# boyuanf/tensorflow_train_distributed

Hardware: AMD Instinct MI355X
Metric: images/sec (whole node) ResNet-50 bf16 MirroredStrategy at 1/2/4/8 MI355X (higher is better)
Workload: dtype bf16; 1 GPU; model=ResNet-50 v1.5, global_batch=1024, per_gpu_batch=1024, image_size=224, parallelism=dp1, optimizer=momentum-SGD 0.9, wd 5e-5, fp32 master, precision=bf16, hipgraph=True

## Files before the change

tensorflow_train_distributed_amd/csrc/kernels/conv3_halo.hip:

```cpp
#include "stream_epi.h"

namespace ttdk {
namespace {
namespace c3 {

constexpr int THR = 512;
constexpr int NW = THR / 64;

struct Pro {
  const bf16_t* x;
  const bf16_t* x2;
  const uint8_t* mask;
  const float* s;
  const float* b;
  bf16_t* side;
  uint8_t* side_mask;
};

__device__ __forceinline__ void load8f(const float* p, float (&d)[8]) {
  const f32x4_t a = *reinterpret_cast<const f32x4_t*>(p), c = *reinterpret_cast<const f32x4_t*>(p + 4);
#pragma unroll
  for (int j = 0; j < 4; ++j) {
    d[j] = a[j];
    d[4 + j] = c[j];
  }
}

template <int CP>
__device__ __forceinline__ int slot_chunk(int q) { return (q >> 3) % CP; }
template <int CP>
__device__ __forceinline__ int slot_pix(int q) { return (q & 7) + 8 * (q / (8 * CP)); }

template <int SCHED>
__device__ __forceinline__ int fresh(int tid) {
  if constexpr (SCHED != 0) {
    asm volatile("" : "+v"(tid));
    __builtin_assume(tid >= 0 && tid < THR);
  }
  return tid;
}

template <int SCHED>
__device__ __forceinline__ void frag_fence() {
  if constexpr (SCHED != 0) __builtin_amdgcn_sched_barrier(0);
}

template <int C, int BN, int TH, int W, int PRO, bool FLIP, int WM, int SCHED>
__global__ __launch_bounds__(THR, 1) void conv3_kernel(Pro pa, const bf16_t* __restrict__ w, EpiParams E, int H,
                                                      int N, int tiles, int nslices) {
  constexpr int BM = TH * W;
  constexpr int HR = TH + 2, HC = W + 2;
  constexpr int CP = C / 8;
  constexpr int KT = 9 * C;
  constexpr int WN = NW / WM;
  constexpr int WR = BM / WM, WC = BN / WN;
  constexpr int TM = WR / 16, TN = WC / 16;
  constexpr int NPIX = HR * HC;
  constexpr int NCH = ((NPIX + 7) / 8) * 8 * CP;
  constexpr int NA = (NCH + THR - 1) / THR;
  constexpr int SB = BN * KT * 2;
  constexpr int REG = ((NPIX * 16 + 255) / 256) * 256;
  constexpr int SH = CP * REG;
  constexpr int PITCH = BN * 2 + 16;
  constexpr int SE = BM * PITCH + NW * 3 * BN * 4;
  constexpr int SAE = SH > SE ? SH : SE;
  static_assert(C % 64 == 0 && BN % 32 == 0 && WR % 16 == 0 && WC % 16 == 0, "tile shape");
  static_assert(THR % (8 * CP) == 0, "fixed channel chunk per thread");
  static_assert(SB + SAE <= 160 * 1024, "LDS budget");
  __shared__ __attribute__((aligned(16))) char smem[SB + SAE];
  char* const sB = smem;
  char* const sA = smem + SB;

  const int b = blockIdx.x;
  const int G = gridDim.x / nslices;
  const int xcd = b & 7, rq = b >> 3;
  const int slice = rq % nslices;
  const int per_xcd = G / 8;
  const int g = xcd * per_xcd + rq / nslices;
  const int n0 = slice * BN;
  const int tid = threadIdx.x, lane = tid & 63, wave = tid >> 6;
  const int wm = wave / WN, wn = wave % WN;
  const int tiles_per_img = H / TH;

  for (int q = tid; q < BN * (KT / 8); q += THR) {
    const int row = q / (KT / 8), kk = q % (KT / 8);
    const int tap = kk / CP, cc = kk % CP;
    const int n = n0 + row;
    const int src_tap = FLIP ? 8 - tap : tap;
    const uint4 v = n < N ? ldg16(w + (static_cast<long long>(n) * 9 + src_tap) * C + cc * 8) : make_uint4(0, 0, 0, 0);
    *reinterpret_cast<uint4*>(sB + (kk >> 3) * (BN * 128) + kmaj_off(row, kk & 7)) = v;
  }

  const int ac = slot_chunk<CP>(tid);
  const bool write_side = slice == 0 && pa.side != nullptr;

  const char* abase[TM];
#pragma unroll
  for (int a = 0; a < TM; ++a) {
    const int i = wm * WR + a * 16 + (lane & 15);
    abase[a] = sA + (lane >> 4) * REG + ((i / W) * HC + (i % W)) * 16;
  }

  uint4 ra[NA], rx[PRO == 2 ? NA : 1];
  uint32_t rm[(NA + 3) / 4];
  auto load_tile = [&](int t) {
    const int img = t / tiles_per_img, h0 = (t % tiles_per_img) * TH;
    const int ft = fresh<SCHED>(tid);
#pragma unroll
    for (int i = 0; i < (NA + 3) / 4; ++i) rm[i] = 0;
#pragma unroll
    for (int i = 0; i < NA; ++i) {
      const int pix = slot_pix<CP>(ft + THR * i);
      const int hr = pix / HC, hc = pix % HC;
      const int h = h0 - 1 + hr, x = hc - 1;
      const bool ok = pix < NPIX && h >= 0 && h < H && x >= 0 && x < W;
      const long long off = ((static_cast<long long>(img) * H + h) * W + x) * C + ac * 8;
      ra[i] = ok ? ldg16(pa.x + off) : make_uint4(0, 0, 0, 0);
      if constexpr (PRO == 2) {
        rx[i] = ok ? ldg16(pa.x2 + off) : make_uint4(0, 0, 0, 0);
        rm[i >> 2] |= static_cast<uint32_t>((ok && pa.mask) ? pa.mask[off >> 3] : 0xffu) << (8 * (i & 3));
      }
    }
  };
  auto stage_tile = [&](int t) {
    const int img = t / tiles_per_img, h0 = (t % tiles_per_img) * TH;
    float k0[8], k1[8], k2[8];
    if constexpr (PRO == 1) {
      load8f(pa.s + ac * 8, k0);
      load8f(pa.b + ac * 8, k1);
    } else if constexpr (PRO == 2) {
      load8f(pa.s + ac * 8, k0);
      load8f(pa.s + C + ac * 8, k1);
      load8f(pa.s + 2 * C + ac * 8, k2);
    }
    const int ft = fresh<SCHED>(tid);
#pragma unroll
    for (int i = 0; i < NA; ++i) {
      const int pix = slot_pix<CP>(ft + THR * i);
      if (ft + THR * i >= NCH) break;
      const int hr = pix / HC, hc = pix % HC;
      const int h = h0 - 1 + hr, x = hc - 1;
      const bool ok = h >= 0 && h < H && x >= 0 && x < W;
      const bool interior = ok && hr >= 1 && hr <= TH;
      const long long off = ((static_cast<long long>(img) * H + h) * W + x) * C + ac * 8;
      uint4 v = ra[i];
      if constexpr (PRO == 1) {
        float f[8];
        unpack8(ra[i], f);
#pragma unroll
        for (int j = 0; j < 8; ++j) f[j] = relu(f[j] * k0[j] + k1[j]);
        v = ok ? pack8(f) : make_uint4(0, 0, 0, 0);
        if (write_side && interior) {
          *reinterpret_cast<uint4*>(pa.side + off) = v;
          if (pa.side_mask) {
            const uint32_t wv[4] = {v.x, v.y, v.z, v.w};
            uint32_t mb = 0;
#pragma unroll
            for (int j = 0; j < 8; ++j) {
              const uint32_t hb = (wv[j >> 1] >> (16 * (j & 1))) & 0xffffu;
              mb |= ((hb & 0x7fffu) != 0 && !(hb & 0x8000u) ? 1u : 0u) << j;
            }
            pa.side_mask[off >> 3] = static_cast<uint8_t>(mb);
          }
        }
      } else if constexpr (PRO == 2) {
        float gq[8], yf[8];
        unpack8(ra[i], gq);
        const uint32_t mb = rm[i >> 2] >> (8 * (i & 3));
#pragma unroll
        for (int j = 0; j < 8; ++j) gq[j] = (mb >> j) & 1u ? gq[j] : 0.f;
        unpack8(rx[i], yf);
#pragma unroll
        for (int j = 0; j < 8; ++j) gq[j] = k0[j] * gq[j] + k1[j] * yf[j] + k2[j];
        v = ok ? pack8(gq) : make_uint4(0, 0, 0, 0);
        if (write_side && interior) *reinterpret_cast<uint4*>(pa.side + off) = v;
      }
      *reinterpret_cast<uint4*>(sA + ac * REG + pix * 16) = v;
    }
  };

  int t = g;
  if (t < tiles) load_tile(t);
  for (; t < tiles; t += G) {
    stage_tile(t);
    __syncthreads();
    if (t + G < tiles) load_tile(t + G);
    f32x4_t acc[TM][TN];
#pragma unroll
    for (int a = 0; a < TM; ++a)
#pragma unroll
      for (int c = 0; c < TN; ++c) acc[a][c] = f32x4_t{0.f, 0.f, 0.f, 0.f};
#pragma unroll
    for (int tap = 0; tap < 9; ++tap) {
      const int tq = (tap / 3) * HC + (tap % 3);
#pragma unroll
      for (int kc = 0; kc < C / 32; ++kc) {
        const int kglob = tap * C + kc * 32;
        const char* pB = sB + (kglob >> 6) * (BN * 128);
        const int kchunk = ((kglob & 63) >> 3) + (lane >> 4);
        bf16x8_t af[TM], bfr[TN];
#pragma unroll
        for (int c = 0; c < TN; ++c) {
          bfr[c] = lds_read_b128(pB + kmaj_off(wn * WC + c * 16 + (lane & 15), kchunk));
          frag_fence<SCHED>();
        }
#pragma unroll
        for (int a = 0; a < TM; ++a) {
          af[a] = lds_read_b128(abase[a] + kc * 4 * REG + tq * 16);
          frag_fence<SCHED>();
        }
#pragma unroll
        for (int a = 0; a < TM; ++a)
#pragma unroll
          for (int c = 0; c < TN; ++c) acc[a][c] = __builtin_amdgcn_mfma_f32_16x16x32_bf16(bfr[c], af[a], acc[a][c], 0, 0, 0);
        frag_fence<SCHED>();
      }
    }
    __syncthreads();
    sepi::stage_acc<TM, TN, WR, WC, PITCH>(sA, acc, wm, wn, lane, epi_alpha(E));
    __syncthreads();
    constexpr int ECPR = BN / 8;
    constexpr int RPP = THR / ECPR;
    const int m0 = t * BM;
    const int c = tid % ECPR, r0 = tid / ECPR;
    const int n = n0 + c * 8;
    const bool nfull = n + 8 <= N;
    const bool vst = nfull && (E.ldo & 7) == 0;
    float bias8[8], s8[8], q8[8], r8[8];
#pragma unroll
    for (int j = 0; j < 8; ++j) {
      bias8[j] = (E.bias && n + j < N) ? E.bias[n + j] : 0.f;
      s8[j] = q8[j] = r8[j] = 0.f;
    }
    const int M = tiles * BM;
    if (E.beta || E.residual || E.by)
      epi_rows<BM, RPP, PITCH, true, 2>(E, sA, c, r0, n, m0, M, N, vst, vst, bias8, s8, q8, r8);
    else
      epi_rows<BM, RPP, PITCH, false>(E, sA, c, r0, n, m0, M, N, vst, vst, bias8, s8, q8, r8);
    if (E.stat)
      sepi::tile_stats<BN, NW, THR, ECPR>(E, reinterpret_cast<float*>(sA + BM * PITCH), s8, q8, r8, c, lane, wave, tid,
                                          n0, N, t);
    else
      __syncthreads();
  }
}

template <int C, int BN, int TH, int W, int PRO, bool FLIP, int WM, int SCHED>
hipError_t launch(const Pro& pa, const bf16_t* w, const EpiParams& E, int Nimg, int H, int N, hipStream_t st) {
  const int nsl = N / BN;
  const int tiles = Nimg * (H / TH);
  int per_xcd = big::device_cus() / (8 * nsl);
  if (per_xcd < 1) per_xcd = 1;
  const int need = ceil_div(tiles, 8);
  if (per_xcd > need) per_xcd = need;
  hipLaunchKernelGGL((conv3_kernel<C, BN, TH, W, PRO, FLIP, WM, SCHED>), dim3(8 * nsl * per_xcd), dim3(THR), 0, st, pa, w,
                     E, H, N, tiles, nsl);
  return hipGetLastError();
}

inline int pick_th(int C, int N, int W, int pro) {
  if (C == 64 && N == 64 && W == 56) return pro == 2 ? 4 : 8;
  return 0;
}

template <int PRO, bool FLIP, int SCHED>
hipError_t dispatch(const Pro& pa, const bf16_t* w, const EpiParams& E, int Nimg, int H, int W, int C, int N,
                    hipStream_t st) {
  if (C == 64 && N == 64 && W == 56) {
    if constexpr (PRO == 2) return launch<64, 64, 4, 56, PRO, FLIP, 2, SCHED>(pa, w, E, Nimg, H, N, st);
    else return launch<64, 64, 8, 56, PRO, FLIP, 4, SCHED>(pa, w, E, Nimg, H, N, st);
  }
  return hipErrorInvalidValue;
}

}

namespace c3s {

constexpr int THR = 512;
constexpr int NW = THR / 64;

__device__ __forceinline__ void dma16(const void* src, uint32_t lds_) {
  const uint32_t lds = __builtin_amdgcn_readfirstlane(lds_);
  unsigned keep;
  asm volatile("s_mov_b32 %0, m0\n\ts_mov_b32 m0, %2\n\ts_nop 0\n\tglobal_load_lds_dwordx4 %1, off\n\ts_mov_b32 m0, %0"
               : "=&s"(keep) : "v"(src), "s"(lds) : "memory");
}
__device__ __forceinline__ uint32_t lds_addr(const char* p) {
  typedef __attribute__((address_space(3))) const char lds_char_t;
  return (uint32_t)(size_t)(lds_char_t*)(p);
}

template <int N>
__device__ __forceinline__ void wait_vm() {
  asm volatile("s_waitcnt vmcnt(%0)" ::"n"(N) : "memory");
}
__device__ __forceinline__ void wait_vm_upto(int n) {
  switch (n) {
    case 1: wait_vm<1>(); break;
    case 2: wait_vm<2>(); break;
    case 3: wait_vm<3>(); break;
    default: wait_vm<0>(); break;
  }
}

template <int C, int BN, int TR, int H, int W, int PRO, bool FLIP, int SCHED>
__global__ __launch_bounds__(THR, 1) void conv3s_kernel(c3::Pro pa, const bf16_t* __restrict__ w, EpiParams E,
                                                       int rows_total, int N, int tiles) {
  constexpr int WM = 2, WN = NW / WM;
  constexpr int BM = TR * W;
  constexpr int WR = BM / WM, WC = BN / WN;
  constexpr int TM = WR / 16, TN = WC / 16;
  constexpr int HS = TR + 4;
  constexpr int HC = W + 2;
  constexpr int NPIX = HS * HC;
  constexpr int CP = C / 8;
  constexpr int NCH = ((NPIX + 7) / 8) * 8 * CP;
  constexpr int NA = (NCH + THR - 1) / THR;
  constexpr int REG = ((NPIX * 16 + 255) / 256) * 256;
  constexpr int SH = CP * REG;
  constexpr int SBT = BN * C * 2;
  constexpr int PITCH = BN * 2 + 16;
  constexpr int SE = BM * PITCH + NW * 3 * BN * 4;
  constexpr int SAE = SH > SE ? SH : SE;
  constexpr int NDMA = SBT / 16 / THR;
  static_assert(PRO != 2 && C % 64 == 0 && BN % (16 * WN) == 0 && WR % 16 == 0 && TR <= H, "tile shape");
  static_assert(THR % (8 * CP) == 0 && SBT % (16 * THR) == 0, "staging / DMA mapping");
  static_assert(SAE + 2 * SBT <= 160 * 1024, "LDS budget");
  __shared__ __attribute__((aligned(16))) char smem[SAE + 2 * SBT];
  char* const sA = smem;
  char* const sBb = smem + SAE;

  const int b = blockIdx.x;
  const int G = gridDim.x;
  const int g = (b & 7) * (G / 8) + (b >> 3);
  const int tid = threadIdx.x, lane = tid & 63, wave = tid >> 6;
  const int wm = wave / WN, wn = wave % WN;
  const int ac = c3::slot_chunk<CP>(tid);
  const bool write_side = pa.side != nullptr;
  const int nimg = rows_total / H;

  const bf16_t* wsrc[NDMA];
#pragma unroll
  for (int i = 0; i < NDMA; ++i) {
    const int L = (i * NW + wave) * 64 + lane;
    const int sub = L / (BN * 8), p = L % (BN * 8), row = p >> 3, j = p & 7;
    const int sc = j ^ ((row >> 1) & 7);
    wsrc[i] = w + static_cast<long long>(row) * 9 * C + (sub * 8 + sc) * 8;
  }
  auto dma_tap = [&](int tap, int buf) {
    const int stap = FLIP ? 8 - tap : tap;
    char* dst = sBb + buf * SBT;
#pragma unroll
    for (int i = 0; i < NDMA; ++i) {
      if constexpr (SCHED != 0) {
        int off = stap * C;
        asm volatile("" : "+s"(off));
        dma16(wsrc[i] + off, lds_addr(dst + (i * NW + wave) * 1024));
      } else {
        const int L = (i * NW + wave) * 64 + lane;
        const int sub = L / (BN * 8), p = L % (BN * 8), row = p >> 3, j = p & 7;
        const int sc = j ^ ((row >> 1) & 7);
        dma16(w + (static_cast<long long>(row) * 9 + stap) * C + (sub * 8 + sc) * 8,
              lds_addr(dst + (i * NW + wave) * 1024));
      }
    }
  };
  struct Geo {
    int i0, h0, n0, n1;
  };
  auto geo = [&](int t) {
    Geo q;
    const int R0 = t * TR, R1 = min(R0 + TR, rows_total);
    q.i0 = R0 / H;
    q.h0 = R0 - q.i0 * H;
    q.n0 = min(R1, (q.i0 + 1) * H) - R0;
    q.n1 = R1 - R0 - q.n0;
    return q;
  };
  auto slot_src = [&](const Geo& q, int s, int& img, int& h, bool& interior) {
    if (s < q.n0 + 2) {
      img = q.i0;
      h = q.h0 - 1 + s;
      interior = s >= 1 && s <= q.n0;
      return true;
    }
    const int u = s - (q.n0 + 2);
    img = q.i0 + 1;
    h = u - 1;
    interior = u >= 1 && u <= q.n1;
    return q.n1 > 0 && u < q.n1 + 2;
  };

  uint4 ra[NA];
  auto load_slot = [&](const Geo& q, int ft, int i) {
    const int qq = ft + THR * i;
    const int pix = c3::slot_pix<CP>(qq);
    const int s = pix / HC, x = pix % HC - 1;
    int img, h;
    bool interior;
    const bool ok = qq < NCH && slot_src(q, s, img, h, interior) && h >= 0 && h < H && x >= 0 && x < W;
    const long long off = ((static_cast<long long>(img) * H + h) * W + x) * C + ac * 8;
    ra[i] = ldg16(ok ? pa.x + off : reinterpret_cast<const bf16_t*>(big::g_zero));
  };
  auto load_tile = [&](int t) {
    const Geo q = geo(t);
    const int ft = c3::fresh<SCHED>(tid);
#pragma unroll
    for (int i = 0; i < NA; ++i) load_slot(q, ft, i);
  };
  auto stage_tile = [&](int t) {
    const Geo q = geo(t);
    float k0[8], k1[8];
    if constexpr (PRO == 1) {
      c3::load8f(pa.s + ac * 8, k0);
      c3::load8f(pa.b + ac * 8, k1);
    }
    const int ft = c3::fresh<SCHED>(tid);
#pragma unroll
    for (int i = 0; i < NA; ++i) {
      const int qq = ft + THR * i;
      if (qq >= NCH) break;
      const int pix = c3::slot_pix<CP>(qq);
      const int s = pix / HC, x = pix % HC - 1;
      int img, h;
      bool interior;
      const bool ok = slot_src(q, s, img, h, interior) && h >= 0 && h < H && x >= 0 && x < W;
      uint4 v = ok ? ra[i] : make_uint4(0, 0, 0, 0);
      if constexpr (PRO == 1) {
        const long long off = ((static_cast<long long>(img) * H + h) * W + x) * C + ac * 8;
        float f[8];
        unpack8(ra[i], f);
#pragma unroll
        for (int j = 0; j < 8; ++j) f[j] = relu(f[j] * k0[j] + k1[j]);
        v = ok ? pack8(f) : make_uint4(0, 0, 0, 0);
        if (write_side && ok && interior) {
          *reinterpret_cast<uint4*>(pa.side + off) = v;
          if (pa.side_mask) {
            const uint32_t wv[4] = {v.x, v.y, v.z, v.w};
            uint32_t mb = 0;
#pragma unroll
            for (int j = 0; j < 8; ++j) {
              const uint32_t hb = (wv[j >> 1] >> (16 * (j & 1))) & 0xffffu;
              mb |= ((hb & 0x7fffu) != 0 && !(hb & 0x8000u) ? 1u : 0u) << j;
            }
            pa.side_mask[off >> 3] = static_cast<uint8_t>(mb);
          }
        }
      }
      *reinterpret_cast<uint4*>(sA + ac * REG + pix * 16) = v;
    }
  };

  int bcur = 0;
  int t = g;
  if (t < tiles) {
    dma_tap(0, 0);
    load_tile(t);
    if constexpr (SCHED != 0) wait_vm<0>();
  }
  for (; t < tiles; t += G) {
    const Geo q = geo(t);
    int abase[TM];
#pragma unroll
    for (int a = 0; a < TM; ++a) {
      const int i = wm * WR + a * 16 + (lane & 15);
      const int j = i / W, col = i % W;
      abase[a] = (lane >> 4) * REG + ((j + (j >= q.n0 ? 2 : 0)) * HC + col) * 16;
    }
    stage_tile(t);
    if constexpr (SCHED == 0) wait_vm<0>();
    __syncthreads();
    const bool more = t + G < tiles;
    f32x4_t acc[TM][TN];
#pragma unroll
    for (int a = 0; a < TM; ++a)
#pragma unroll
      for (int c = 0; c < TN; ++c) acc[a][c] = f32x4_t{0.f, 0.f, 0.f, 0.f};
    constexpr int HPT = 2;
    static_assert(HPT * 8 >= NA, "the halo loads are all retired by the wait of the last tap");
    const Geo qn = geo(SCHED != 0 && more ? t + G : t);
#pragma unroll(SCHED != 0 ? 9 : 1)
    for (int tap = 0; tap < 9; ++tap) {
      const int bnext = bcur ^ 1;
      if (tap < 8) dma_tap(tap + 1, bnext);
      else if (more) dma_tap(0, bnext);
      const int h0 = tap * HPT < NA ? tap * HPT : NA, h1 = h0 + HPT < NA ? h0 + HPT : NA;
      if constexpr (SCHED != 0) {
        if (more) {
          const int ft = c3::fresh<SCHED>(tid);
#pragma unroll
          for (int i = h0; i < h1; ++i) load_slot(qn, ft, i);
        }
      }
      const char* sBc = sBb + bcur * SBT;
      const int tq = ((tap / 3) * HC + (tap % 3)) * 16;
#pragma unroll
      for (int kc = 0; kc < C / 32; ++kc) {
        const int kglob = kc * 32;
        const char* pB = sBc + (kglob >> 6) * (BN * 128);
        const int kchunk = ((kglob & 63) >> 3) + (lane >> 4);
        bf16x8_t af[TM], bfr[TN];
#pragma unroll
        for (int c = 0; c < TN; ++c) {
          bfr[c] = lds_read_b128(pB + kmaj_off(wn * WC + c * 16 + (lane & 15), kchunk));
          c3::frag_fence<SCHED>();
        }
#pragma unroll
        for (int a = 0; a < TM; ++a) {
          af[a] = lds_read_b128(sA + abase[a] + kc * 4 * REG + tq);
          c3::frag_fence<SCHED>();
        }
#pragma unroll
        for (int a = 0; a < TM; ++a)
#pragma unroll
          for (int c = 0; c < TN; ++c) acc[a][c] = __builtin_amdgcn_mfma_f32_16x16x32_bf16(bfr[c], af[a], acc[a][c], 0, 0, 0);
        c3::frag_fence<SCHED>();
      }
      if constexpr (SCHED != 0) wait_vm_upto(more ? h1 - h0 : 0);
      else wait_vm<0>();
      __syncthreads();
      bcur = bnext;
    }
    sepi::stage_acc<TM, TN, WR, WC, PITCH>(sA, acc, wm, wn, lane, epi_alpha(E));
    if constexpr (SCHED == 0)
      if (more) load_tile(t + G);
    __syncthreads();
    constexpr int ECPR = BN / 8;
    constexpr int RPP = THR / ECPR;
    const int m0 = t * BM;
    const int c = tid % ECPR, r0 = tid / ECPR;
    const int n = c * 8;
    const bool vst = (E.ldo & 7) == 0;
    float bias8[8], s8[8], q8[8], r8[8];
#pragma unroll
    for (int j = 0; j < 8; ++j) {
      bias8[j] = E.bias ? E.bias[n + j] : 0.f;
      s8[j] = q8[j] = r8[j] = 0.f;
    }
    const int M = rows_total * W;
    if (E.beta || E.residual || E.by)
      epi_rows<BM, RPP, PITCH, true, 2>(E, sA, c, r0, n, m0, M, N, vst, vst, bias8, s8, q8, r8);
    else
      epi_rows<BM, RPP, PITCH, false>(E, sA, c, r0, n, m0, M, N, vst, vst, bias8, s8, q8, r8);
    if (E.stat)
      sepi::tile_stats<BN, NW, THR, ECPR>(E, reinterpret_cast<float*>(sA + BM * PITCH), s8, q8, r8, c, lane, wave, tid,
                                          0, N, t);
    else
      __syncthreads();
    (void)nimg;
  }
}

template <int PRO, bool FLIP, int SCHED>
hipError_t launch(const c3::Pro& pa, const bf16_t* w, const EpiParams& E, int Nimg, int N, hipStream_t st) {
  const int rows = Nimg * 28;
  const int tiles = ceil_div(rows, 8);
  int G = big::device_cus() / 8 * 8;
  if (G < 8) G = 8;
  const int need = ceil_div(tiles, 8) * 8;
  if (G > need) G = need;
  hipLaunchKernelGGL((conv3s_kernel<128, 128, 8, 28, 28, PRO, FLIP, SCHED>), dim3(G), dim3(THR), 0, st, pa, w, E, rows,
                     N, tiles);
  return hipGetLastError();
}

inline bool fits(int H, int W, int C, int N, int pro) { return C == 128 && N == 128 && H == 28 && W == 28 && pro != 2; }

}
}
}

using namespace ttdk;

namespace {
int& conv3_s3_flag() {
  static int on = getenv_int("TTD_CONV3_S3", 1);
  return on;
}
int& conv3_sched_flag() {
  static int on = getenv_int("TTD_CONV3_SCHED", 1);
  return on;
}
}

TTDK_EXPORT int ttdk_set_conv3_sched(int on) {
  const int old = conv3_sched_flag();
  conv3_sched_flag() = on ? 1 : 0;
  return old;
}

TTDK_EXPORT int ttdk_set_conv3_s3(int on) {
  const int old = conv3_s3_flag();
  conv3_s3_flag() = on;
  return old;
}

TTDK_EXPORT int ttdk_conv3_rows(int H, int W, int C, int N, int pro) {
  if (conv3_s3_flag() && c3s::fits(H, W, C, N, pro)) return 8 * W;
  const int th = c3::pick_th(C, N, W, pro);
  return (th && H % th == 0) ? th * W : 0;
}

TTDK_EXPORT int ttdk_conv3_halo(const bf16_t* x, const bf16_t* x2, const uint8_t* mask_in, const float* s,
                                const float* b, bf16_t* side, uint8_t* side_mask, int pro, int flip, const bf16_t* w,
                                int Nimg, int H, int W, int C, int N, const TtdkEpilogue* epi, hipStream_t st) {
  const int sched = conv3_sched_flag();
  if (ttdk_conv3_rows(H, W, C, N, pro) == 8 * W && c3s::fits(H, W, C, N, pro)) {
    if ((reinterpret_cast<uintptr_t>(x) & 15) || (reinterpret_cast<uintptr_t>(w) & 15)) return hipErrorInvalidValue;
    const EpiParams e = to_epi(epi);
    if (e.mode != 0 || e.remap || e.bH || e.ldo != N || e.residual || e.by2) return hipErrorInvalidValue;
    if (pro == 1 && (!s || !b)) return hipErrorInvalidValue;
    if (side_mask && pro != 1) return hipErrorInvalidValue;
    const c3::Pro pa{x, nullptr, nullptr, s, b, side, side_mask};
#define C3S_CASE(P_, F_)              \
  if (pro == P_ && (flip != 0) == F_) \
    return sched ? c3s::launch<P_, F_, 1>(pa, w, e, Nimg, N, st) : c3s::launch<P_, F_, 0>(pa, w, e, Nimg, N, st);
    C3S_CASE(0, false)
    C3S_CASE(0, true)
    C3S_CASE(1, false)
#undef C3S_CASE
    return hipErrorInvalidValue;
  }
  const int th = c3::pick_th(C, N, W, pro);
  if (!th || H % th || (reinterpret_cast<uintptr_t>(x) & 15) || pro < 0 || pro > 2) return hipErrorInvalidValue;
  const EpiParams e = to_epi(epi);
  if (e.mode != 0 || e.remap || e.bH || e.ldo != N || e.residual || e.by2) return hipErrorInvalidValue;
  if (pro == 1 && (!s || !b)) return hipErrorInvalidValue;
  if (pro == 2 && (!s || !x2)) return hipErrorInvalidValue;
  if (side_mask && pro != 1) return hipErrorInvalidValue;
  const c3::Pro pa{x, x2, mask_in, s, b, side, side_mask};
#define C3_CASE(P_, F_)                                                           \
  if (pro == P_ && (flip != 0) == F_)                                             \
    return sched ? c3::dispatch<P_, F_, 1>(pa, w, e, Nimg, H, W, C, N, st)        \
                 : c3::dispatch<P_, F_, 0>(pa, w, e, Nimg, H, W, C, N, st);
  C3_CASE(0, false)
  C3_CASE(1, false)
  C3_CASE(0, true)
  C3_CASE(2, true)
#undef C3_CASE
  return hipErrorInvalidValue;
}
```

tensorflow_train_distributed_amd/csrc/kernels/stream_epi.h:

```cpp
#pragma once

#include "gemm_conv.h"

namespace ttdk {
namespace {
namespace sepi {

template <int TM, int TN, int WR, int WC, int PITCH>
__device__ __forceinline__ void stage_acc(char* sS, const f32x4_t (&acc)[TM][TN], int wm, int wn, int lane,
                                          float alpha) {
  const int gq4 = lane >> 4, i16 = lane & 15;
#pragma unroll
  for (int a = 0; a < TM; ++a)
#pragma unroll
    for (int c = 0; c < TN; ++c) {
      const int r = wm * WR + a * 16 + i16, cc = wn * WC + c * 16 + 4 * gq4;
      const f32x4_t v = acc[a][c] * alpha;
      *reinterpret_cast<uint2*>(sS + r * PITCH + cc * 2) = make_uint2(pack_bf16x2(v[0], v[1]), pack_bf16x2(v[2], v[3]));
    }
}

template <int BN, int NW, int THR, int ECPR>
__device__ __forceinline__ void tile_stats(const EpiParams& E, float* red, float (&s8)[8], float (&q8)[8],
                                           float (&r8)[8], int c, int lane, int wave, int tid, int n0, int N, long long t) {
  static_assert(ECPR <= 64, "one chunk column per lane group");
#pragma unroll
  for (int j = 0; j < 8; ++j) {
#pragma unroll
    for (int o = ECPR; o < 64; o <<= 1) {
      s8[j] += __shfl_xor(s8[j], o, 64);
      q8[j] += __shfl_xor(q8[j], o, 64);
      if (E.stat2) r8[j] += __shfl_xor(r8[j], o, 64);
    }
  }
  if (lane < ECPR) {
#pragma unroll
    for (int j = 0; j < 8; ++j) {
      red[(wave * 3 + 0) * BN + c * 8 + j] = s8[j];
      red[(wave * 3 + 1) * BN + c * 8 + j] = q8[j];
      red[(wave * 3 + 2) * BN + c * 8 + j] = r8[j];
    }
  }
  __syncthreads();
  for (int t2 = tid; t2 < BN; t2 += THR) {
    if (n0 + t2 < N) {
      float ss = 0.f, qq = 0.f, rr = 0.f;
#pragma unroll
      for (int k = 0; k < NW; ++k) {
        ss += red[(k * 3 + 0) * BN + t2];
        qq += red[(k * 3 + 1) * BN + t2];
        rr += red[(k * 3 + 2) * BN + t2];
      }
      E.stat[(t * 2 + 0) * N + n0 + t2] = ss;
      E.stat[(t * 2 + 1) * N + n0 + t2] = qq;
      if (E.stat2) {
        E.stat2[(t * 2 + 0) * N + n0 + t2] = ss;
        E.stat2[(t * 2 + 1) * N + n0 + t2] = rr;
      }
    }
  }
  __syncthreads();
}

}
}
}
```

tensorflow_train_distributed_amd/ops/gemm.py:

```python
from __future__ import annotations

import ctypes

import torch

from . import _lib, _plan

ACT_NONE, ACT_RELU, ACT_GELU, ACT_TANH, ACT_DGELU = 0, 1, 2, 3, 4

import os as _os
_LOG = [] if _os.environ.get("TTD_GEMM_LOG") else None


def gemm_log(reset=False):
    out = list(_LOG or [])
    if reset and _LOG is not None:
        _LOG.clear()
    return out


def _log(kind, M, N, K, splits=1):
    if _LOG is not None:
        _LOG.append((kind, int(M), int(N), int(K), int(splits)))
    _lib.label((kind, int(M), int(N), int(K)))
# ... 74 lines not shown
    if out.dtype == torch.float32:
        splits = effective_splits(K, splits)
        if splits > 1:
            if not out.is_contiguous():
                raise ValueError("split-K output must be contiguous")
            ws = torch.empty((splits, M, N), dtype=torch.float32, device=a.device)
            _lib.call("ttdk_gemm_bf16_splitk", a.data_ptr(), lda, a_kmajor, b.data_ptr(), ldb, b_kmajor, M, N, K,
                      splits, ws.data_ptr(), out.data_ptr(), beta, float(alpha), int(tile[0]), int(tile[1]),
                      _lib.stream())
            return out
        e = _epi(out, mode=2, beta=beta, alpha=alpha)
    else:
        e = _epi(out, bias=bias, residual=residual, act=act, beta=beta, alpha=alpha, aux=aux, stat=stat)
    _lib.call("ttdk_gemm_bf16", a.data_ptr(), lda, a_kmajor, b.data_ptr(), ldb, b_kmajor, M, N, K, 1,
              tile[0], tile[1], ctypes.byref(e), _lib.stream())
    return out


_lib.register({"ttdk_gemm4w_bf16": [_lib.P, _lib.L, _lib.P, _lib.L, _lib.I, _lib.I, _lib.I, _lib.E, _lib.P],
               "ttdk_set_g4_sched": [_lib.I], "ttdk_set_g4_group": [_lib.I],
               "ttdk_set_g4_stagger": [_lib.I]})


def set_g4_stagger(v: int) -> int:
    return int(_lib.query("ttdk_set_g4_stagger", int(v)))


def set_g4_group(v: int) -> int:
    return int(_lib.query("ttdk_set_g4_group", int(v)))


def set_g4_sched(v: int) -> int:
    return int(_lib.query("ttdk_set_g4_sched", int(v)))


def gemm4w(a, b, *, out=None, bias=None, act=ACT_NONE, residual=None, beta=0, alpha=1.0, aux=None):
    _check2d(a, torch.bfloat16, "a")
    _check2d(b, torch.bfloat16, "b")
    M, K = a.shape
    N, Kb = b.shape
    if K != Kb:
        raise ValueError("gemm4w inner dims differ: %d vs %d" % (K, Kb))
    if out is None:
        out = torch.empty((M, N), dtype=torch.bfloat16, device=a.device)
    e = _epi(out, bias=bias, residual=residual, act=act, beta=beta, alpha=alpha, aux=aux)
    _log("gemm4w", M, N, K, 1)
    _lib.call("ttdk_gemm4w_bf16", a.data_ptr(), a.stride(0), b.data_ptr(), b.stride(0), M, N, K, ctypes.byref(e),
              _lib.stream())
    return out


_lib.register({"ttdk_gemm_bf16_batched": [_lib.P, _lib.L, _lib.L, _lib.I, _lib.P, _lib.L, _lib.L, _lib.I, _lib.P,
                                          _lib.L, _lib.L, _lib.I, _lib.I, _lib.I, _lib.I, _lib.I, _lib.P],
               "ttdk_gemm_f32_batched": [_lib.P, _lib.L, _lib.L, _lib.I, _lib.P, _lib.L, _lib.L, _lib.I, _lib.P,
                                         _lib.L, _lib.L, _lib.I, _lib.I, _lib.I, _lib.I, _lib.P]})


def gemm_batched(a, b, *, trans_a=False, trans_b=False, out_dtype=torch.float32):
    if a.dim() != 3 or b.dim() != 3 or a.shape[0] != b.shape[0]:
        raise ValueError("gemm_batched needs [B, ., .] operands with equal batch, got %s and %s"
                         % (tuple(a.shape), tuple(b.shape)))
    a = a.contiguous()
    b = b.contiguous()
    Bt = a.shape[0]
    M, K = (a.shape[2], a.shape[1]) if trans_a else (a.shape[1], a.shape[2])
    Kb, N = (b.shape[2], b.shape[1]) if trans_b else (b.shape[1], b.shape[2])
    if K != Kb:
        raise ValueError("gemm_batched inner dims differ: %d vs %d" % (K, Kb))
    _log("gemm_batched", M, N, K, Bt)
    if a.dtype == torch.float32 and b.dtype == torch.float32:
        out = torch.empty((Bt, M, N), dtype=torch.float32, device=a.device)
        _lib.call("ttdk_gemm_f32_batched", a.data_ptr(), a.stride(1), a.stride(0), int(trans_a), b.data_ptr(),
                  b.stride(1), b.stride(0), int(trans_b), out.data_ptr(), N, M * N, M, N, K, Bt, _lib.stream())
        return out
    _check(a, torch.bfloat16, "a")
    _check(b, torch.bfloat16, "b")
    out = torch.empty((Bt, M, N), dtype=out_dtype, device=a.device)
    _lib.call("ttdk_gemm_bf16_batched", a.data_ptr(), a.stride(1), a.stride(0), 0 if trans_a else 1, b.data_ptr(),
              b.stride(1), b.stride(0), 1 if trans_b else 0, out.data_ptr(), N, M * N,
              1 if out_dtype == torch.float32 else 0, M, N, K, Bt, _lib.stream())
    return out


def wgrad_bias_ok(M, N, K, splits) -> bool:
    if M % 8 or N % 8 or K % 64:
        return False
    if int(_lib.query("ttdk_gemm_wgrad_bias_ws", int(M), int(N), int(K), int(splits))) < 0:
        return False
    kt = K // 64
    return -(-kt // _plan.clamp_splits(kt, int(splits))) >= 16


def gemm_wgrad_bias(dy, x, out, bias_out, splits=1, beta=0, alpha=1.0):
    _check2d(dy, torch.bfloat16, "dy")
    _check2d(x, torch.bfloat16, "x")
    K, M = dy.shape
    K2, N = x.shape
    if K != K2:
        raise ValueError("gemm_wgrad_bias: token dims differ (%d vs %d)" % (K, K2))
    if tuple(out.shape) != (M, N) or out.dtype != torch.float32 or not out.is_contiguous():
        raise ValueError("gemm_wgrad_bias: out must be a contiguous fp32 [%d, %d]" % (M, N))
    if bias_out.numel() != M or bias_out.dtype != torch.float32 or not bias_out.is_contiguous():
        raise ValueError("gemm_wgrad_bias: bias_out must be a contiguous fp32 [%d]" % M)
    nws = int(_lib.query("ttdk_gemm_wgrad_bias_ws", M, N, K, int(splits)))
    if nws < 0:
        raise ValueError("gemm_wgrad_bias: shape %dx%dx%d not on the 256-wide kernel" % (M, N, K))
    ws = torch.empty(nws, dtype=torch.float32, device=dy.device)
    _log("wgrad_bias", M, N, K, splits)
    _lib.call("ttdk_gemm_wgrad_bias", dy.data_ptr(), dy.stride(0), x.data_ptr(), x.stride(0), M, N, K, int(splits),
              ws.data_ptr(), out.data_ptr(), int(beta), float(alpha), bias_out.data_ptr(), _lib.stream())
    return out, bias_out


def gemm4t(dy, x, out=None, bias_out=None, *, splits=1, beta=0, alpha=1.0):
    _check2d(dy, torch.bfloat16, "dy")
    _check2d(x, torch.bfloat16, "x")
    K, M = dy.shape
    K2, N = x.shape
    if K != K2:
        raise ValueError("gemm4t: token dims differ (%d vs %d)" % (K, K2))
    if out is None:
        out = torch.empty((M, N), dtype=torch.float32, device=dy.device)
    if tuple(out.shape) != (M, N) or out.dtype != torch.float32 or not out.is_contiguous():
        raise ValueError("gemm4t: out must be a contiguous fp32 [%d, %d]" % (M, N))
    if bias_out is not None and (bias_out.numel() != M or bias_out.dtype != torch.float32
                                 or not bias_out.is_contiguous()):
        raise ValueError("gemm4t: bias_out must be a contiguous fp32 [%d]" % M)
    nws = int(_lib.query("ttdk_gemm4t_ws", M, N, K, int(splits)))
    if nws < 0:
        raise ValueError("gemm4t does not take M=%d N=%d K=%d (K a multiple of 64 >= 128, M / N multiples "
                         "of 8, operands < 2 GiB, TTD_G4T on)" % (M, N, K))
    ws = torch.empty(max(nws, 1), dtype=torch.float32, device=dy.device)
    _log("gemm4t", M, N, K, splits)
    _lib.call("ttdk_gemm4t_wgrad", dy.data_ptr(), dy.stride(0), x.data_ptr(), x.stride(0), M, N, K, int(splits),
              ws.data_ptr(), out.data_ptr(), int(beta), float(alpha), _lib.ptr(bias_out), _lib.stream())
    return out


_C3 = _os.environ.get("TTD_CONV3", "1") != "0"


_lib.register({"ttdk_set_conv3_s3": [_lib.I]})


def set_conv3_s3(on: bool) -> bool:
    return bool(_lib.query("ttdk_set_conv3_s3", 1 if on else 0))


_lib.register({"ttdk_set_conv3_sched": [_lib.I]})


def set_conv3_sched(new: bool) -> bool:
    return bool(_lib.query("ttdk_set_conv3_sched", 1 if new else 0))


def conv3_rows(H, W, C, N, pro=0):
    return int(_lib.query("ttdk_conv3_rows", int(H), int(W), int(C), int(N), int(pro))) if _C3 else 0


def conv3_halo(x, w, *, prologue=None, flip=False, out=None, stat=False, bn_stat=None):
    _check(x, torch.bfloat16, "x")
    _check(w, torch.bfloat16, "w")
    Nimg, H, W, C = x.shape
    Co = w.shape[0]
    if tuple(w.shape) != (Co, 3, 3, C):
        raise ValueError("conv3_halo: filter must be [%d, 3, 3, %d], got %s" % (Co, C, tuple(w.shape)))
    pro_code = 0 if prologue is None else {"bn_fwd": 1, "bn_bwd": 2}.get(prologue[0], -1)
    bm = conv3_rows(H, W, C, Co, max(pro_code, 0))
    if not bm:
        raise ValueError("conv3_halo: shape %s -> %d not compiled in" % (tuple(x.shape), Co))
    if out is None:
        out = torch.empty((Nimg, H, W, Co), dtype=torch.bfloat16, device=x.device)
    T = -(-Nimg * H * W // bm)
    partial = None
    by = bmask = None
    if stat or bn_stat is not None:
        partial = torch.empty((T, 2, Co), dtype=torch.float32, device=x.device)
    if bn_stat is not None:
        by, bmask = bn_stat
        _check(by, torch.bfloat16, "bn_stat y")
    e = _epi(out, ldo=Co, stat=partial, by=by, bmask=bmask)
    P = _lib.ptr
    pro, x2, mask_in, s, b, side, side_mask = 0, None, None, None, None, None, None
    if prologue is not None:
        if prologue[0] == "bn_fwd":
            _, s, b, side, side_mask = prologue
            pro = 1
        elif prologue[0] == "bn_bwd":
            _, x2, mask_in, s, side = prologue
            pro = 2
        else:
            raise ValueError("unknown prologue %r" % (prologue[0],))
    _log("c3_%s" % ("dgrad" if flip else "fwd"), Nimg * H * W, Co, 9 * C)
    _lib.call("ttdk_conv3_halo", x.data_ptr(), P(x2), P(mask_in), P(s), P(b), P(side), P(side_mask), pro, int(flip),
              w.data_ptr(), Nimg, H, W, C, Co, ctypes.byref(e), _lib.stream())
    if partial is not None:
        return out, partial, T
    return out


def gemm_f32(a, b, *, trans_a=False, trans_b=False, out=None, bias=None, beta=0):
    _check2d(a, torch.float32, "a")
    _check2d(b, torch.float32, "b")
    M, K = (a.shape[1], a.shape[0]) if trans_a else a.shape
    Kb, N = (b.shape[1], b.shape[0]) if trans_b else b.shape
    if K != Kb:
        raise ValueError("gemm inner dims differ: %d vs %d" % (K, Kb))
    if out is None:
        if beta:
            raise ValueError("beta=1 needs an out tensor")
        out = torch.empty((M, N), dtype=torch.float32, device=a.device)
    elif out.dtype != torch.float32 or tuple(out.shape) != (M, N) or out.stride(-1) != 1:
        raise ValueError("gemm_f32 out must be fp32 [%d, %d] row-major" % (M, N))
    if bias is not None:
        _check(bias, torch.float32, "bias")
    _log("gemm_f32_%s%s" % ("t" if trans_a else "n", "t" if trans_b else "n"), M, N, K, 1)
    _lib.call("ttdk_gemm_f32", a.data_ptr(), a.stride(0), int(trans_a), b.data_ptr(), b.stride(0), int(trans_b),
              out.data_ptr(), out.stride(0), _lib.ptr(bias), int(bool(beta)), M, N, K, _lib.stream())
    return out


BIG_WGRAD_WGS = int(_os.environ.get("TTD_WGRAD_WGS", "128"))


def gemm_wgrad_splits(M, N, K, target_blocks=1024, min_ktiles=8, big_wgs=None):
    bbn = big_bn(M, N, K)
    if bbn:
        tiles = -(-M // 256) * -(-N // bbn)
        return max(1, min((K // 64) // 32, -(-(big_wgs or BIG_WGRAD_WGS) // tiles)))
    bm, bn = _plan.pick_tile(M, N)
    tiles = -(-M // bm) * -(-N // bn)
    ktiles = -(-K // 64)
    return max(1, min(ktiles // min_ktiles, -(-target_blocks // tiles)))


def conv_geom(x_shape, w_shape, stride, padding, dilation=(1, 1)):
    N, H, W, C = x_shape
    K, R, S, Cw = w_shape
    if C != Cw:
        raise ValueError("channel mismatch %d vs %d" % (C, Cw))
    sh, sw = stride
    ph, pw = padding
    dh, dw = dilation
    P = (H + 2 * ph - dh * (R - 1) - 1) // sh + 1
    Q = (W + 2 * pw - dw * (S - 1) - 1) // sw + 1
    g = _lib.ConvGeom(N, H, W, C, K, R, S, P, Q, sh, sw, ph, pw, dh, dw)
    return g


def pw_rows(N, K, dma=False):
    return int(_lib.query("ttdk_pw_rows", int(N), int(K), int(bool(dma))))


_PW = _os.environ.get("TTD_PW", "1") != "0"


def pw_ok(M, N, K):
    return _PW and pw_rows(N, K) > 0 and N * K <= 65536


def pw_wgrad_fusable(M, N, K, dma=True):
    return _PW and int(_lib.query("ttdk_pw_wgrad_slabs", int(M), int(N), int(K), int(bool(dma)), 0)) > 0


def pw_conv(x, w, *, prologue=None, out=None, stat=False, beta=0, residual=None, bn_stat=None, bn_stat2=None,
            beta_s2=None, wgrad=None, max_wgs=0, fold_stream=None, keep=None):
    _check(x, torch.bfloat16, "x")
    _check(w, torch.bfloat16, "w")
    K = x.shape[-1]
    M = x.numel() // K
    N = w.shape[0]
    if w.numel() != N * K:
        raise ValueError("pw_conv: weight must be [N, K] = [%d, %d] (got %s)" % (N, K, tuple(w.shape)))
    dma = bool(beta or bn_stat is not None) and residual is None and bn_stat2 is None
    bm = pw_rows(N, K, dma)
    if not bm:
        raise ValueError("pw_conv: N=%d K=%d not handled by the streaming kernel" % (N, K))
    if out is None:
        out = torch.empty(tuple(x.shape[:-1]) + (N,), dtype=torch.bfloat16, device=x.device)
    T = -(-M // bm)
    partial = partial2 = None
    by = bmask = by2 = None
    if stat or bn_stat is not None:
        partial = torch.empty((T, 2, N), dtype=torch.float32, device=x.device)
    if bn_stat is not None:
        by, bmask = bn_stat
        _check(by, torch.bfloat16, "bn_stat y")
        if bn_stat2 is not None:
            by2 = bn_stat2
            partial2 = torch.empty((T, 2, N), dtype=torch.float32, device=x.device)
    e = _epi(out, ldo=N, beta=beta, residual=residual, stat=partial, by=by, bmask=bmask, by2=by2, stat2=partial2,
             beta_s2=beta_s2 if beta else None)
    P = _lib.ptr
    pro, x2, mask_in, s, b, rs, rb, side, side_mask = 0, None, None, None, None, None, None, None, None
    if prologue is not None:
        if prologue[0] == "bn_fwd":
            _, s, b, x2, rs, rb, side, side_mask = prologue
            pro = 1
        elif prologue[0] == "bn_bwd":
            _, x2, mask_in, s, side = prologue
            pro = 2
        else:
            raise ValueError("pw_conv: unknown prologue %r" % (prologue[0],))
    _log("pw_%s" % ("fwd" if pro != 2 else "dgrad"), M, N, K)
    if wgrad is not None:
        xw, dw = wgrad[0], wgrad[1]
# ... 571 lines not shown
```

Baseline: 15800 images/sec.

## Prefetch epilogue BN-backward inputs during late conv3 taps in data-gradient kernels

Adds a FEED variant of the halo conv3 kernels used for data gradients that issues the epilogue's global loads (by activations and bmask) early, during the later MMA taps and the accumulator staging, so they overlap with compute. A specialized epilogue then masks, stores and accumulates the BN statistics from these register-held batches. The goal is to hide the epilogue's memory latency, at the cost of extra registers and more complex vmcnt accounting. The variant is on by default and controlled by an env flag.

```diff
diff --git a/tensorflow_train_distributed_amd/csrc/kernels/conv3_halo.hip b/tensorflow_train_distributed_amd/csrc/kernels/conv3_halo.hip
--- a/tensorflow_train_distributed_amd/csrc/kernels/conv3_halo.hip
+++ b/tensorflow_train_distributed_amd/csrc/kernels/conv3_halo.hip
@@ -45,7 +45,7 @@
   if constexpr (SCHED != 0) __builtin_amdgcn_sched_barrier(0);
 }
 
-template <int C, int BN, int TH, int W, int PRO, bool FLIP, int WM, int SCHED>
+template <int C, int BN, int TH, int W, int PRO, bool FLIP, int WM, int SCHED, int FEED>
 __global__ __launch_bounds__(THR, 1) void conv3_kernel(Pro pa, const bf16_t* __restrict__ w, EpiParams E, int H,
                                                       int N, int tiles, int nslices) {
   constexpr int BM = TH * W;
@@ -179,12 +179,22 @@
     }
   };
 
+  constexpr int ECPR = BN / 8;
+  constexpr int RPP = THR / ECPR;
+  constexpr int NR = (BM + RPP - 1) / RPP;
+  constexpr int FA = NR >= 6 ? 3 : 2, FTAP = 6;
+  static_assert(FEED == 0 || (FLIP && SCHED != 0), "feeding epilogue: data gradients under SCHED 1");
+  const int M = tiles * BM;
+
   int t = g;
   if (t < tiles) load_tile(t);
   for (; t < tiles; t += G) {
     stage_tile(t);
     __syncthreads();
     if (t + G < tiles) load_tile(t + G);
+    const int m0 = t * BM;
+    sepi::FeedBatch<FA> fa;
+    sepi::FeedBatch<NR - FA> fb;
     f32x4_t acc[TM][TN];
 #pragma unroll
     for (int a = 0; a < TM; ++a)
@@ -195,6 +205,12 @@
       const int tq = (tap / 3) * HC + (tap % 3);
 #pragma unroll
       for (int kc = 0; kc < C / 32; ++kc) {
+        if constexpr (FEED != 0) {
+          if (tap == FTAP && kc == 0) {
+            const int ft = fresh<SCHED>(tid);
+            sepi::feed_batch_load<BM, RPP, FA>(fa, E, 0, ft / ECPR, m0, M, n0 + (ft % ECPR) * 8);
+          }
+        }
         const int kglob = tap * C + kc * 32;
         const char* pB = sB + (kglob >> 6) * (BN * 128);
         const int kchunk = ((kglob & 63) >> 3) + (lane >> 4);
@@ -217,13 +233,12 @@
       }
     }
     __syncthreads();
+    const int fe = fresh<SCHED>(tid);
+    const int c = fe % ECPR, r0 = fe / ECPR;
+    const int n = n0 + c * 8;
     sepi::stage_acc<TM, TN, WR, WC, PITCH>(sA, acc, wm, wn, lane, epi_alpha(E));
+    if constexpr (FEED != 0) sepi::feed_batch_load<BM, RPP, NR - FA>(fb, E, FA, r0, m0, M, n);
     __syncthreads();
-    constexpr int ECPR = BN / 8;
-    constexpr int RPP = THR / ECPR;
-    const int m0 = t * BM;
-    const int c = tid % ECPR, r0 = tid / ECPR;
-    const int n = n0 + c * 8;
     const bool nfull = n + 8 <= N;
     const bool vst = nfull && (E.ldo & 7) == 0;
     float bias8[8], s8[8], q8[8], r8[8];
@@ -232,8 +247,10 @@
       bias8[j] = (E.bias && n + j < N) ? E.bias[n + j] : 0.f;
       s8[j] = q8[j] = r8[j] = 0.f;
     }
-    const int M = tiles * BM;
-    if (E.beta || E.residual || E.by)
+    if constexpr (FEED != 0) {
+      sepi::feed_batch_rows<BM, RPP, PITCH, FA>(fa, E, sA, 0, c, r0, m0, M, n, s8, q8);
+      sepi::feed_batch_rows<BM, RPP, PITCH, NR - FA>(fb, E, sA, FA, c, r0, m0, M, n, s8, q8);
+    } else if (E.beta || E.residual || E.by)
       epi_rows<BM, RPP, PITCH, true, 2>(E, sA, c, r0, n, m0, M, N, vst, vst, bias8, s8, q8, r8);
     else
       epi_rows<BM, RPP, PITCH, false>(E, sA, c, r0, n, m0, M, N, vst, vst, bias8, s8, q8, r8);
@@ -245,7 +262,7 @@
   }
 }
 
-template <int C, int BN, int TH, int W, int PRO, bool FLIP, int WM, int SCHED>
+template <int C, int BN, int TH, int W, int PRO, bool FLIP, int WM, int SCHED, int FEED>
 hipError_t launch(const Pro& pa, const bf16_t* w, const EpiParams& E, int Nimg, int H, int N, hipStream_t st) {
   const int nsl = N / BN;
   const int tiles = Nimg * (H / TH);
@@ -253,8 +270,8 @@
   if (per_xcd < 1) per_xcd = 1;
   const int need = ceil_div(tiles, 8);
   if (per_xcd > need) per_xcd = need;
-  hipLaunchKernelGGL((conv3_kernel<C, BN, TH, W, PRO, FLIP, WM, SCHED>), dim3(8 * nsl * per_xcd), dim3(THR), 0, st, pa, w,
-                     E, H, N, tiles, nsl);
+  hipLaunchKernelGGL((conv3_kernel<C, BN, TH, W, PRO, FLIP, WM, SCHED, FEED>), dim3(8 * nsl * per_xcd), dim3(THR), 0, st,
+                     pa, w, E, H, N, tiles, nsl);
   return hipGetLastError();
 }
 
@@ -263,12 +280,12 @@
   return 0;
 }
 
-template <int PRO, bool FLIP, int SCHED>
+template <int PRO, bool FLIP, int SCHED, int FEED>
 hipError_t dispatch(const Pro& pa, const bf16_t* w, const EpiParams& E, int Nimg, int H, int W, int C, int N,
                     hipStream_t st) {
   if (C == 64 && N == 64 && W == 56) {
-    if constexpr (PRO == 2) return launch<64, 64, 4, 56, PRO, FLIP, 2, SCHED>(pa, w, E, Nimg, H, N, st);
-    else return launch<64, 64, 8, 56, PRO, FLIP, 4, SCHED>(pa, w, E, Nimg, H, N, st);
+    if constexpr (PRO == 2) return launch<64, 64, 4, 56, PRO, FLIP, 2, SCHED, FEED>(pa, w, E, Nimg, H, N, st);
+    else return launch<64, 64, 8, 56, PRO, FLIP, 4, SCHED, FEED>(pa, w, E, Nimg, H, N, st);
   }
   return hipErrorInvalidValue;
 }
@@ -304,7 +321,7 @@
   }
 }
 
-template <int C, int BN, int TR, int H, int W, int PRO, bool FLIP, int SCHED>
+template <int C, int BN, int TR, int H, int W, int PRO, bool FLIP, int SCHED, int FEED>
 __global__ __launch_bounds__(THR, 1) void conv3s_kernel(c3::Pro pa, const bf16_t* __restrict__ w, EpiParams E,
                                                        int rows_total, int N, int tiles) {
   constexpr int WM = 2, WN = NW / WM;
@@ -452,6 +469,14 @@
     }
   };
 
+  constexpr int ECPR = BN / 8;
+  constexpr int RPP = THR / ECPR;
+  constexpr int NR = (BM + RPP - 1) / RPP;
+  constexpr int FA = 3, FTAP = 9 - FA;
+  static_assert(NR > FA, "two batches");
+  static_assert(FEED == 0 || (FLIP && SCHED != 0), "feeding epilogue: data gradients under SCHED 1");
+  const int M = rows_total * W;
+
   int bcur = 0;
   int t = g;
   if (t < tiles) {
@@ -472,6 +497,8 @@
     if constexpr (SCHED == 0) wait_vm<0>();
     __syncthreads();
     const bool more = t + G < tiles;
+    sepi::FeedBatch<1> fa[FA];
+    sepi::FeedBatch<NR - FA> fb;
     f32x4_t acc[TM][TN];
 #pragma unroll
     for (int a = 0; a < TM; ++a)
@@ -479,6 +506,8 @@
       for (int c = 0; c < TN; ++c) acc[a][c] = f32x4_t{0.f, 0.f, 0.f, 0.f};
     constexpr int HPT = 2;
     static_assert(HPT * 8 >= NA, "the halo loads are all retired by the wait of the last tap");
+    static_assert(HPT * FTAP >= NA, "no tap issues both halo and feeding loads (wait_vm_upto takes 0 .. 3)");
+    const int m0 = t * BM;
     const Geo qn = geo(SCHED != 0 && more ? t + G : t);
 #pragma unroll(SCHED != 0 ? 9 : 1)
     for (int tap = 0; tap < 9; ++tap) {
@@ -493,6 +522,13 @@
           for (int i = h0; i < h1; ++i) load_slot(qn, ft, i);
         }
       }
+      const int nfeed = (FEED != 0 && tap >= FTAP) ? 2 : 0;
+      if constexpr (FEED != 0) {
+        if (tap >= FTAP) {
+          const int ft = c3::fresh<SCHED>(tid);
+          sepi::feed_batch_load<BM, RPP, 1>(fa[tap - FTAP], E, tap - FTAP, ft / ECPR, m0, M, (ft % ECPR) * 8);
+        }
+      }
       const char* sBc = sBb + bcur * SBT;
       const int tq = ((tap / 3) * HC + (tap % 3)) * 16;
 #pragma unroll
@@ -517,20 +553,19 @@
           for (int c = 0; c < TN; ++c) acc[a][c] = __builtin_amdgcn_mfma_f32_16x16x32_bf16(bfr[c], af[a], acc[a][c], 0, 0, 0);
         c3::frag_fence<SCHED>();
       }
-      if constexpr (SCHED != 0) wait_vm_upto(more ? h1 - h0 : 0);
+      if constexpr (SCHED != 0) wait_vm_upto((more ? h1 - h0 : 0) + nfeed);
       else wait_vm<0>();
       __syncthreads();
       bcur = bnext;
     }
+    const int fe = c3::fresh<SCHED>(tid);
+    const int c = fe % ECPR, r0 = fe / ECPR;
+    const int n = c * 8;
     sepi::stage_acc<TM, TN, WR, WC, PITCH>(sA, acc, wm, wn, lane, epi_alpha(E));
+    if constexpr (FEED != 0) sepi::feed_batch_load<BM, RPP, NR - FA>(fb, E, FA, r0, m0, M, n);
     if constexpr (SCHED == 0)
       if (more) load_tile(t + G);
     __syncthreads();
-    constexpr int ECPR = BN / 8;
-    constexpr int RPP = THR / ECPR;
-    const int m0 = t * BM;
-    const int c = tid % ECPR, r0 = tid / ECPR;
-    const int n = c * 8;
     const bool vst = (E.ldo & 7) == 0;
     float bias8[8], s8[8], q8[8], r8[8];
 #pragma unroll
@@ -538,8 +573,11 @@
       bias8[j] = E.bias ? E.bias[n + j] : 0.f;
       s8[j] = q8[j] = r8[j] = 0.f;
     }
-    const int M = rows_total * W;
-    if (E.beta || E.residual || E.by)
+    if constexpr (FEED != 0) {
+#pragma unroll
+      for (int k = 0; k < FA; ++k) sepi::feed_batch_rows<BM, RPP, PITCH, 1>(fa[k], E, sA, k, c, r0, m0, M, n, s8, q8);
+      sepi::feed_batch_rows<BM, RPP, PITCH, NR - FA>(fb, E, sA, FA, c, r0, m0, M, n, s8, q8);
+    } else if (E.beta || E.residual || E.by)
       epi_rows<BM, RPP, PITCH, true, 2>(E, sA, c, r0, n, m0, M, N, vst, vst, bias8, s8, q8, r8);
     else
       epi_rows<BM, RPP, PITCH, false>(E, sA, c, r0, n, m0, M, N, vst, vst, bias8, s8, q8, r8);
@@ -552,7 +590,7 @@
   }
 }
 
-template <int PRO, bool FLIP, int SCHED>
+template <int PRO, bool FLIP, int SCHED, int FEED>
 hipError_t launch(const c3::Pro& pa, const bf16_t* w, const EpiParams& E, int Nimg, int N, hipStream_t st) {
   const int rows = Nimg * 28;
   const int tiles = ceil_div(rows, 8);
@@ -560,8 +598,8 @@
   if (G < 8) G = 8;
   const int need = ceil_div(tiles, 8) * 8;
   if (G > need) G = need;
-  hipLaunchKernelGGL((conv3s_kernel<128, 128, 8, 28, 28, PRO, FLIP, SCHED>), dim3(G), dim3(THR), 0, st, pa, w, E, rows,
-                     N, tiles);
+  hipLaunchKernelGGL((conv3s_kernel<128, 128, 8, 28, 28, PRO, FLIP, SCHED, FEED>), dim3(G), dim3(THR), 0, st, pa, w, E,
+                     rows, N, tiles);
   return hipGetLastError();
 }
 
@@ -582,6 +620,16 @@
   static int on = getenv_int("TTD_CONV3_SCHED", 1);
   return on;
 }
+int& conv3_feed_flag() {
+  static int on = getenv_int("TTD_CONV3_FEED", 1);
+  return on;
+}
+}
+
+TTDK_EXPORT int ttdk_set_conv3_feed(int on) {
+  const int old = conv3_feed_flag();
+  conv3_feed_flag() = on ? 1 : 0;
+  return old;
 }
 
 TTDK_EXPORT int ttdk_set_conv3_sched(int on) {
@@ -613,9 +661,11 @@
     if (pro == 1 && (!s || !b)) return hipErrorInvalidValue;
     if (side_mask && pro != 1) return hipErrorInvalidValue;
     const c3::Pro pa{x, nullptr, nullptr, s, b, side, side_mask};
+    if (pro == 0 && flip && sched && conv3_feed_flag() && sepi::feed_case(e))
+      return c3s::launch<0, true, 1, 1>(pa, w, e, Nimg, N, st);
 #define C3S_CASE(P_, F_)              \
   if (pro == P_ && (flip != 0) == F_) \
-    return sched ? c3s::launch<P_, F_, 1>(pa, w, e, Nimg, N, st) : c3s::launch<P_, F_, 0>(pa, w, e, Nimg, N, st);
+    return sched ? c3s::launch<P_, F_, 1, 0>(pa, w, e, Nimg, N, st) : c3s::launch<P_, F_, 0, 0>(pa, w, e, Nimg, N, st);
     C3S_CASE(0, false)
     C3S_CASE(0, true)
     C3S_CASE(1, false)
@@ -630,10 +680,14 @@
   if (pro == 2 && (!s || !x2)) return hipErrorInvalidValue;
   if (side_mask && pro != 1) return hipErrorInvalidValue;
   const c3::Pro pa{x, x2, mask_in, s, b, side, side_mask};
-#define C3_CASE(P_, F_)                                                           \
-  if (pro == P_ && (flip != 0) == F_)                                             \
-    return sched ? c3::dispatch<P_, F_, 1>(pa, w, e, Nimg, H, W, C, N, st)        \
-                 : c3::dispatch<P_, F_, 0>(pa, w, e, Nimg, H, W, C, N, st);
+  if (flip && sched && conv3_feed_flag() && sepi::feed_case(e)) {
+    if (pro == 0) return c3::dispatch<0, true, 1, 1>(pa, w, e, Nimg, H, W, C, N, st);
+    if (pro == 2) return c3::dispatch<2, true, 1, 1>(pa, w, e, Nimg, H, W, C, N, st);
+  }
+#define C3_CASE(P_, F_)                                                        \
+  if (pro == P_ && (flip != 0) == F_)                                          \
+    return sched ? c3::dispatch<P_, F_, 1, 0>(pa, w, e, Nimg, H, W, C, N, st)  \
+                 : c3::dispatch<P_, F_, 0, 0>(pa, w, e, Nimg, H, W, C, N, st);
   C3_CASE(0, false)
   C3_CASE(1, false)
   C3_CASE(0, true)
diff --git a/tensorflow_train_distributed_amd/csrc/kernels/stream_epi.h b/tensorflow_train_distributed_amd/csrc/kernels/stream_epi.h
--- a/tensorflow_train_distributed_amd/csrc/kernels/stream_epi.h
+++ b/tensorflow_train_distributed_amd/csrc/kernels/stream_epi.h
@@ -62,6 +62,71 @@
   __syncthreads();
 }
 
+template <int NRW>
+struct FeedBatch {
+  uint4 y[NRW];
+  uint32_t mb[NRW];
+};
+
+template <int BM, int RPP, int NRW>
+__device__ __forceinline__ void feed_batch_load(FeedBatch<NRW>& f, const EpiParams& E, int k0, int r0, int m0, int M,
+                                                int n) {
+  const long long o0 = static_cast<long long>(m0 + r0 + k0 * RPP) * E.ldo + n;
+  const long long step = static_cast<long long>(RPP) * E.ldo;
+  const bf16_t* yp = E.by + o0;
+  const uint8_t* mp = E.bmask + (o0 >> 3);
+#pragma unroll
+  for (int u = 0; u < NRW; ++u) {
+    const int r = r0 + (k0 + u) * RPP;
+    const bool ok = r < BM && m0 + r < M;
+    f.y[u] = ldg16(ok ? yp : reinterpret_cast<const bf16_t*>(big::g_zero));
+    f.mb[u] = *((ok && E.bmask) ? mp : reinterpret_cast<const uint8_t*>(big::g_zero));
+    yp += step;
+    mp += step >> 3;
+  }
+}
+
+template <int BM, int RPP, int PITCH, int NRW>
+__device__ __forceinline__ void feed_batch_rows(const FeedBatch<NRW>& f, const EpiParams& E, const char* smem, int k0,
+                                                int c, int r0, int m0, int M, int n, float (&s8)[8], float (&q8)[8]) {
+  const long long step = static_cast<long long>(RPP) * E.ldo;
+  bf16_t* op = static_cast<bf16_t*>(E.out) + static_cast<long long>(m0 + r0 + k0 * RPP) * E.ldo + n;
+  uint4 sv[NRW];
+#pragma unroll
+  for (int u = 0; u < NRW; ++u) {
+    const int r = r0 + (k0 + u) * RPP;
+    sv[u] = *reinterpret_cast<const uint4*>(smem + (r < BM ? r : r0) * PITCH + c * 16);
+  }
+#pragma unroll
+  for (int u = 0; u < NRW; ++u, op += step) {
+    __builtin_amdgcn_sched_barrier(0);
+    const int r = r0 + (k0 + u) * RPP;
+    if (r >= BM || m0 + r >= M) break;
+    float v[8], yv[8];
+    unpack8(sv[u], v);
+    const uint32_t mb = E.bmask ? f.mb[u] : 0xffu;
+#pragma unroll
+    for (int j = 0; j < 8; ++j) {
+      v[j] += 0.f;
+      v[j] = (mb >> j) & 1u ? v[j] : 0.f;
+    }
+    const uint4 packed = pack8(v);
+    *reinterpret_cast<uint4*>(op) = packed;
+    unpack8(packed, v);
+    unpack8(f.y[u], yv);
+#pragma unroll
+    for (int j = 0; j < 8; ++j) {
+      s8[j] += v[j];
+      q8[j] += v[j] * yv[j];
+    }
+  }
+}
+
+inline bool feed_case(const EpiParams& E) {
+  return E.by && !E.by2 && !E.bias && !E.residual && !E.beta && !E.aux && E.act == kActNone && !E.remap &&
+         (E.ldo & 7) == 0;
+}
+
 }
 }
 }
diff --git a/tensorflow_train_distributed_amd/ops/gemm.py b/tensorflow_train_distributed_amd/ops/gemm.py
--- a/tensorflow_train_distributed_amd/ops/gemm.py
+++ b/tensorflow_train_distributed_amd/ops/gemm.py
@@ -250,6 +250,13 @@
 
 def set_conv3_sched(new: bool) -> bool:
     return bool(_lib.query("ttdk_set_conv3_sched", 1 if new else 0))
+
+
+_lib.register({"ttdk_set_conv3_feed": [_lib.I]})
+
+
+def set_conv3_feed(new: bool) -> bool:
+    return bool(_lib.query("ttdk_set_conv3_feed", 1 if new else 0))
 
 
 def conv3_rows(H, W, C, N, pro=0):
```

Measured after the change: 15970 images/sec (median of 6 runs). 1.01x the previous value.
